# mjuvela/SOC

Measured on AMD Instinct MI355X. Metric: photon packets/sec, higher is better.
Workload: dtype f32

## Files before the change

soc_amd/csrc/soc_brick.hip:

```cpp
#include "soc_walk.h"
#include "soc_ltree.h"

#include <cstdio>
#include <algorithm>
#include <chrono>
#include <cstdlib>
#include <cstring>
#include <vector>

#include "soc_lbricks.h"

#define SOC_BRICK_T 256

#if defined(SOC_BRICK_PROF)
__device__ unsigned long long g_soc_prof[24];
#define SOC_PROF_DECL unsigned int prof_[8] = { 0, 0, 0, 0, 0, 0, 0, 0 }, dprof_[8] = { 0, 0, 0, 0, 0, 0, 0, 0 };  unsigned long long tprof_[8] = { 0, 0, 0, 0, 0, 0, 0, 0 }, tlast_ = __builtin_readcyclecounter()
#define SOC_PROF_T(i) do { const unsigned long long t_ = __builtin_readcyclecounter();  tprof_[i] += t_ - tlast_;  tlast_ = t_; } while (0)
#define SOC_PROF_ENTRY const unsigned long long tentry_ = __builtin_readcyclecounter()
#define SOC_PROF_SINCE_ENTRY(i) do { tprof_[i] += tlast_ - tentry_; } while (0)
#define SOC_PROF(i, n) do { prof_[i] += (unsigned int)(n); } while (0)
#define SOC_DPROF(i, n) do { dprof_[i] += (unsigned int)(n); } while (0)
#define SOC_PROF_FLUSH do { if ((threadIdx.x & 63) == 0) for (int i_ = 0; i_ < 8; i_++) atomicAdd(&g_soc_prof[16 + i_], (unsigned long long)dprof_[i_]); \
                            if ((threadIdx.x & 63) == 0) for (int i_ = 0; i_ < 8; i_++) atomicAdd(&g_soc_prof[i_], (unsigned long long)prof_[i_]); \
                            if ((threadIdx.x & 63) == 0) for (int i_ = 0; i_ < 8; i_++) atomicAdd(&g_soc_prof[8 + i_], tprof_[i_]); } while (0)
// ... 1766 lines not shown
{
    if ((int)blockIdx.x >= nsort) {
        const int e = (int)blockIdx.x - nsort, l = e >> 4, part = e & 15;
        const int start = A.admit[1 + 3 * l], n = A.admit[2 + 3 * l];
        if (n > 0) {
            const int dst = A.admit[3 + 3 * l];
            for (int i = part * SOC_BRICK_T + threadIdx.x; i < n; i += 16 * SOC_BRICK_T) A.idq_next[dst + i] = (uint32_t)(start + i);
        }
        return;
    }
    if ((int)blockIdx.x >= *A.ndesc) return;
    const SocDesc D = A.desc[blockIdx.x];
    for (int j = threadIdx.x; j < D.count; j += SOC_BRICK_T) {
        const uint32_t key = A.keyq[D.start + j];
        if (key < (uint32_t)A.NB) A.idq_next[A.off[key] + A.posq[D.start + j]] = A.idq[D.start + j];
    }
}


#include "soc_devbuf.h"

#define BCHK(call)                          \
    do {                                    \
        hipError_t e_ = (call);             \
        if (e_ != hipSuccess) return e_;    \
    } while (0)

struct SocBrickBuffers {
    DevBuf<SocPk2> pk, park;
    DevBuf<float2> kopt;
    DevBuf<uint32_t> idq[2], keyq, posq;
    DevBuf<SocSimPack> pack;
    DevBuf<int> hist, off, ndesc, total, admit;
    DevBuf<SocDesc> desc[2];
};

template <typename T>
static hipError_t upload(DevBuf<T> &d, const std::vector<T> &v, hipStream_t st)
{
    BCHK(d.reset(v.size(), st));
    return hipMemcpy(d, v.data(), v.size() * sizeof(T), hipMemcpyHostToDevice);
}

struct SocOctBricks {
    bool valid = false;
    int  NB = 0, CAP = 0;
    size_t cells = 0, leaves = 0;
    DevBuf<float2> DS;
    DevBuf<int> bcell, bbase;
};

struct SocLBricksDev {
    bool valid = false, failed = false;
    int  NB = 0, cap = 0, max_slots = 0;
    size_t cells = 0, slots = 0;
    DevBuf<SocLBrick> lbr;
    DevBuf<float> btree;
    DevBuf<int> bcell, bbase, rbrick;
};

struct SocSweepState {
    SocBrickBuffers bb;
    SocOctBricks ob;
    SocLBricksDev lb;
};

SocSweepState *soc_sweep_new() { return new SocSweepState(); }
void soc_sweep_delete(SocSweepState *sw) { delete sw; }
void soc_sweep_invalidate(SocSweepState *sw) { sw->ob.valid = false;  sw->lb.valid = false;  sw->lb.failed = false; }

static hipError_t soc_oct_build(SocOctBricks &ob, const SocGrid &G, int CAP, hipStream_t st, bool verbose)
{
    if (ob.valid && ob.CAP == CAP && ob.cells == (size_t)G.CELLS) return hipSuccess;
    ob.valid = false;
    std::vector<float> D((size_t)G.CELLS);
    BCHK(hipStreamSynchronize(st));
    BCHK(hipMemcpy(D.data(), G.DENS, (size_t)G.CELLS * 4, hipMemcpyDeviceToHost));
    SocOctBuilder B(G.NX, G.NY, G.NZ, G.LEVELS, G.CELLS, G.LCELLS, G.OFF, D.data(), CAP);
    B.build();
    const int NB = (int)B.bbase.size() - 1;
    if (NB < 1 || NB >= (1 << (32 - SOC_SLOT_BITS))) return hipErrorNotSupported;
    std::vector<float2> DS((size_t)G.CELLS);
    for (size_t i = 0; i < (size_t)G.CELLS; i++) { float y;  memcpy(&y, &B.slotmap[i], 4);  DS[i] = make_float2(D[i], y); }
    BCHK(upload(ob.DS, DS, st));
    BCHK(upload(ob.bcell, B.bcell, st));
    BCHK(upload(ob.bbase, B.bbase, st));
    ob.NB = NB;  ob.CAP = CAP;  ob.cells = (size_t)G.CELLS;  ob.leaves = B.bcell.size();
    ob.valid = true;
    if (verbose)
        fprintf(stderr, "soc_brick: hierarchy of %d cells, %zu leaves -> %d bricks of <= %d leaves (mean %.0f)\n",
                G.CELLS, ob.leaves, NB, CAP, (double)ob.leaves / NB);
    return hipSuccess;
}

static hipError_t soc_lb_build(SocLBricksDev &lb, const SocGrid &G, int cap, hipStream_t st, bool verbose)
{
    if (lb.cap == cap && lb.cells == (size_t)G.CELLS) {
        if (lb.valid) return hipSuccess;
        if (lb.failed) return hipErrorNotSupported;
    }
    lb.valid = false;  lb.failed = false;
    lb.cap = cap;  lb.cells = (size_t)G.CELLS;
    std::vector<float> D((size_t)G.CELLS);
    BCHK(hipStreamSynchronize(st));
    BCHK(hipMemcpy(D.data(), G.DENS, (size_t)G.CELLS * 4, hipMemcpyDeviceToHost));
    SocLBricksHost H;
    const bool built = (G.LEVELS == 1) ? soc_cbricks_build(G.NX, G.NY, G.NZ, D.data(), soc_cart_edge(cap), H)
                                       : soc_lbricks_build(G.NX, G.NY, G.NZ, G.LEVELS, G.LCELLS, G.OFF, D.data(), cap, H);
    if (!built || H.bricks.size() >= (1u << 20)) {
        lb.failed = true;
        return hipErrorNotSupported;
    }
    const int NB = (int)H.bricks.size();
    std::vector<int> bbase((size_t)NB + 1);
    for (int b = 0; b < NB; b++) bbase[b] = H.bricks[b].base;
    bbase[NB] = (int)H.btree.size();
    BCHK(upload(lb.lbr, H.bricks, st));
    BCHK(upload(lb.btree, H.btree, st));
    BCHK(upload(lb.bcell, H.bcell, st));
    BCHK(upload(lb.bbase, bbase, st));
    BCHK(upload(lb.rbrick, H.rbrick, st));
    lb.NB = NB;  lb.max_slots = H.max_slots;  lb.slots = H.btree.size();
    lb.valid = true;
    if (verbose)
        fprintf(stderr, "soc_brick: %s of %d cells -> %d brick-local hierarchies of <= %d cells (largest %d, mean %.0f)\n",
                (G.LEVELS == 1) ? "grid" : "hierarchy", G.CELLS, NB, cap, H.max_slots, (double)G.CELLS / NB);
    return hipSuccess;
}


typedef void (*SocPassFn)(const SocGrid, const SocSimPack *, const SocBrickArgs, const int, const int);
static const SocPassFn soc_brick_pass_fns[3][2][2][4] = {
    { { { soc_brick_pass<0, 0, 0, 0, 0>, soc_brick_pass<0, 0, 0, 0, 1>, soc_brick_pass<0, 0, 0, 0, 2>, soc_brick_pass<0, 0, 0, 0, 3> },
        { soc_brick_pass<0, 0, 0, 1, 0>, soc_brick_pass<0, 0, 0, 1, 1>, soc_brick_pass<0, 0, 0, 1, 2>, soc_brick_pass<0, 0, 0, 1, 3> } },
      { { soc_brick_pass<0, 0, 1, 0, 0>, soc_brick_pass<0, 0, 1, 0, 1>, soc_brick_pass<0, 0, 1, 0, 2>, soc_brick_pass<0, 0, 1, 0, 3> },
        { soc_brick_pass<0, 0, 1, 1, 0>, soc_brick_pass<0, 0, 1, 1, 1>, soc_brick_pass<0, 0, 1, 1, 2>, soc_brick_pass<0, 0, 1, 1, 3> } } },
    { { { soc_brick_pass<1, 0, 0, 0, 0>, soc_brick_pass<1, 0, 0, 0, 1>, soc_brick_pass<1, 0, 0, 0, 2>, soc_brick_pass<1, 0, 0, 0, 3> },
        { soc_brick_pass<1, 0, 0, 1, 0>, soc_brick_pass<1, 0, 0, 1, 1>, soc_brick_pass<1, 0, 0, 1, 2>, soc_brick_pass<1, 0, 0, 1, 3> } },
      { { soc_brick_pass<1, 0, 1, 0, 0>, soc_brick_pass<1, 0, 1, 0, 1>, soc_brick_pass<1, 0, 1, 0, 2>, soc_brick_pass<1, 0, 1, 0, 3> },
        { soc_brick_pass<1, 0, 1, 1, 0>, soc_brick_pass<1, 0, 1, 1, 1>, soc_brick_pass<1, 0, 1, 1, 2>, soc_brick_pass<1, 0, 1, 1, 3> } } },
    { { { soc_brick_pass<1, 1, 0, 0, 0>, soc_brick_pass<1, 1, 0, 0, 1>, soc_brick_pass<1, 1, 0, 0, 2>, soc_brick_pass<1, 1, 0, 0, 3> },
        { soc_brick_pass<1, 1, 0, 1, 0>, soc_brick_pass<1, 1, 0, 1, 1>, soc_brick_pass<1, 1, 0, 1, 2>, soc_brick_pass<1, 1, 0, 1, 3> } },
      { { soc_brick_pass<1, 1, 1, 0, 0>, soc_brick_pass<1, 1, 1, 0, 1>, soc_brick_pass<1, 1, 1, 0, 2>, soc_brick_pass<1, 1, 1, 0, 3> },
        { soc_brick_pass<1, 1, 1, 1, 0>, soc_brick_pass<1, 1, 1, 1, 1>, soc_brick_pass<1, 1, 1, 1, 2>, soc_brick_pass<1, 1, 1, 1, 3> } } } };
static const SocPassFn soc_lbrick_pass_fns[4][5] = {
    { soc_lbrick_pass<0, 0>, soc_lbrick_pass<0, 1>, soc_lbrick_pass<0, 2>, soc_lbrick_pass<0, 3>, soc_lbrick_pass<0, 4> },
    { soc_lbrick_pass<1, 0>, soc_lbrick_pass<1, 1>, soc_lbrick_pass<1, 2>, soc_lbrick_pass<1, 3>, soc_lbrick_pass<1, 4> },
    { soc_lbrick_pass<2, 0>, soc_lbrick_pass<2, 1>, soc_lbrick_pass<2, 2>, soc_lbrick_pass<2, 3>, soc_lbrick_pass<2, 4> },
    { soc_lbrick_pass<3, 0>, soc_lbrick_pass<3, 1>, soc_lbrick_pass<3, 2>, soc_lbrick_pass<3, 3>, soc_lbrick_pass<3, 4> } };
static const SocPassFn soc_lbrick_pass_ali_fns[2] = { soc_lbrick_pass_ali<0>, soc_lbrick_pass_ali<1> };
static const SocPassFn soc_lbrick_pass_abu_fns[4] = { soc_lbrick_pass_abu<0>, soc_lbrick_pass_abu<1>, nullptr, soc_lbrick_pass_abu<3> };
static const SocPassFn soc_lbrick_pass_flt_fns[4] = { soc_lbrick_pass_flt<0>, soc_lbrick_pass_flt<1>, soc_lbrick_pass_flt<2>, soc_lbrick_pass_flt<3> };
static const SocPassFn soc_lbrick_pass_ali_flt_fns[2] = { soc_lbrick_pass_ali_flt<0>, soc_lbrick_pass_ali_flt<1> };
static const SocPassFn soc_lray_pass_fns[2][2][2] = { { { soc_lray_pass<0, 0, 0>, soc_lray_pass<0, 1, 0> }, { soc_lray_pass<1, 0, 0>, soc_lray_pass<1, 1, 0> } },
                                                      { { soc_lray_pass<0, 0, 1>, soc_lray_pass<0, 1, 1> }, { soc_lray_pass<1, 0, 1>, soc_lray_pass<1, 1, 1> } } };

static const SocPassFn soc_lray_pass_flt_fns[2][2] = { { soc_lray_pass<0, 0, 0, 1>, soc_lray_pass<0, 1, 0, 1> }, { soc_lray_pass<1, 0, 0, 1>, soc_lray_pass<1, 1, 0, 1> } };

static SocPassFn pass_kernel(const SocSweepPlan &pl)
{
    const bool flt = (pl.form == 3) && pl.octree && !pl.dbl;
    if (pl.rays)      return flt ? soc_lray_pass_flt_fns[pl.hpx][pl.hpsky] : soc_lray_pass_fns[pl.octree ? 0 : 1][pl.hpx][pl.hpsky];
    if (flt && pl.abu) return nullptr;
    if (flt)          return pl.ali ? soc_lbrick_pass_ali_flt_fns[pl.wint] : soc_lbrick_pass_flt_fns[pl.wint];
    if (pl.form == 3 && pl.abu) return soc_lbrick_pass_abu_fns[pl.wint];
    if (pl.form == 3) return pl.ali ? soc_lbrick_pass_ali_fns[pl.wint] : soc_lbrick_pass_fns[pl.wint][pl.kind];
    return soc_brick_pass_fns[pl.octree + pl.dbl][pl.abu][pl.wint][pl.kind];
}

static hipError_t check_sca(const SocSim *S, int nlaunch, const SocVariant &V, const SocSca *sca)
{
    if (!sca) return hipSuccess;
    if (sca->NDIR == 0 || V.abu || V.wint) return hipErrorNotSupported;
    for (int l = 0; l < nlaunch; l++) {
        const int k = S[l].SCAKIND - 1;
        if ((k != SOC_SCA_PB && k != SOC_SCA_PS && k != SOC_SCA_CL && k != SOC_SCA_HP) || S[l].NDUST > 1 || S[l].BINS < 1 || !S[l].OUT) return hipErrorNotSupported;
        if ((k == SOC_SCA_PB || k == SOC_SCA_PS) && !S[l].DSC) return hipErrorNotSupported;
        if ((k == SOC_SCA_HP) && (!S[l].HPBG || (S[l].HPBG_WEIGHTED && !S[l].HPBGP))) return hipErrorNotSupported;
        if ((k == SOC_SCA_CL) != (S[l].SOURCE == SOC_SOURCE_CL)) return hipErrorInvalidValue;
    }
    return hipSuccess;
}

static hipError_t plan_sweep(SocSweepPlan &pl, const SocGrid &G, const SocSim *S, int nlaunch, const SocVariant &V,
                             const SocBrickTune &tune, const SocSca *sca, bool lb_ok)
{
    const bool cart = lb_ok && sca && soc_brick_cart(G, V);
    bool xab = false;
    for (int l = 0; l < nlaunch; l++) xab = xab || (S[l].XAB != nullptr);
    const bool lt = cart || (lb_ok && soc_brick_local(G, V, tune) && !(V.abu && xab));
    pl = soc_grid_plan(lt ? 3 : V.octree ? 2 : 1, 0, V);
    pl.rays = sca != nullptr;
    pl.hpx = sca && sca->NDIR < 0;
    for (int l = 0; l < nlaunch && sca; l++) pl.hpsky = pl.hpsky || (S[l].SCAKIND == SOC_SCA_HP + 1);
    const auto pick = [](int t, int d) { return (t > 0) ? t : d; };
    pl.T = pick(tune.T, 512);
    if (lt) {
        pl.P = pick(tune.P, 16384);
        pl.KCAP = pick(tune.KCAP, 64);
        pl.FTH = pick(tune.FTH, 16);
        pl.CTH = pick(tune.CTH, 8);
        pl.TAIL = pick(tune.TAIL, 32);
        pl.PARK = pick(tune.park, 4096);
        pl.slow_every = tune.slow_every;
    } else {
        pl.P = pick(tune.P, V.octree ? 4096 : 2048);
        pl.KCAP = pick(tune.KCAP, V.octree ? 32 : 48);
        pl.FTH = pick(tune.FTH, V.octree ? 16 : 24);
        pl.CTH = pick(tune.CTH, pl.FTH);
        pl.TAIL = pick(tune.TAIL, 0);
        pl.CAP = pick(tune.CAP, 6144);
    }
    if (pl.T < 64 || pl.T > 1024 || (pl.T & 63) || pl.P < 1 || pl.P > SOC_LBRICK_PMAX || pl.KCAP < 1) return hipErrorInvalidValue;
    pl.EQ = 2;
    if (!lt) {
        if (sca || V.wint == 2) return hipErrorNotSupported;
        for (int l = 0; l < nlaunch; l++) if (S[l].ROISAVE) return hipErrorNotSupported;
        if (pl.T > 512 || pl.P > SOC_BRICK_PMAX || pl.CAP < 8 || pl.CAP > (1 << SOC_SLOT_BITS)) return hipErrorInvalidValue;
        return hipSuccess;
    }
    bool int_only = !sca && (V.wint == 1);
    for (int l = 0; l < nlaunch && int_only; l++)
        for (int m = 0; m < l; m++) if (S[m].INT == S[l].INT && S[m].TW != S[l].TW) { int_only = false;  break; }
    bool ali = !sca && (V.wint != 2);
    for (int l = 0; l < nlaunch; l++) ali = ali && (S[l].SOURCE == SOC_SOURCE_CL) && (S[l].XAB != nullptr) && (S[l].XAB == S[0].XAB);
    if (ali) int_only = false;
    pl.wint = int_only ? 3 : V.wint;
    pl.ali = ali;
    const int cedge = soc_cart_default_edge(G);
    const int cap_abu = (V.wint && !int_only) ? 3456 : 4352;
    pl.capl = (tune.CAP > 0) ? tune.CAP : cart ? cedge * cedge * cedge : (sca ? 17408 : V.abu ? cap_abu : (ali ? (V.wint ? 3456 : 4352) : (V.wint == 2 ? 2944 : (V.wint && !int_only) ? 5888 : 8704)));
    if (pl.capl < 8 || pl.capl > 36864) return hipErrorInvalidValue;
    pl.EQ = 3;
    for (int l = 0; l < nlaunch; l++) pl.roi = pl.roi || (S[l].ROISAVE && S[l].ROI);
    if (pl.roi) {
        for (int l = 0; l < nlaunch; l++) if (!(S[l].ROISAVE && S[l].ROI) || S[l].MIRROR) return hipErrorNotSupported;
        pl.EQ = 4;
    }
    return hipSuccess;
}

static hipError_t build_bricks(SocBrickArgs &A, const SocSweepPlan &pl, SocSweepState &sw, const SocGrid &G, int LB, hipStream_t st, bool verbose)
{
    A = SocBrickArgs{};
    A.LB = LB;
    A.ev_brick = -1;
    A.T = pl.T;  A.P = pl.P;  A.KCAP = pl.KCAP;  A.FTH = pl.FTH;  A.CTH = pl.CTH;  A.CAP = pl.CAP;  A.TAIL = pl.TAIL;  A.PARK = pl.PARK;
    A.EQ = pl.EQ;  A.slow_every = pl.slow_every;
    A.LT = (pl.form == 3);  A.int_only = (pl.wint == 3);  A.ali = pl.ali;  A.roi_on = pl.roi;
    if (pl.form == 1) {
        const int B = 1 << LB;
        A.NBX = (G.NX + B - 1) / B;  A.NBY = (G.NY + B - 1) / B;  A.NBZ = (G.NZ + B - 1) / B;
        A.NB = A.NBX * A.NBY * A.NBZ;
        return (A.NB > (1 << 18)) ? hipErrorNotSupported : hipSuccess;
    }
    int k = 1;
    while ((1 << k) <= std::max(G.NX, std::max(G.NY, G.NZ))) k++;
    A.sib_thr = ldexpf(1.0f, k - 29);
    A.kexp = k - 30;
    if (pl.form == 3) {
        BCHK(soc_lb_build(sw.lb, G, pl.capl, st, verbose));
        const SocLBricksDev &lb = sw.lb;
        A.NB = lb.NB;
        A.CAP = (lb.max_slots + 63) & ~63;
        A.lbr = lb.lbr;  A.btree = lb.btree;  A.bcell = lb.bcell;  A.bbase = lb.bbase;  A.rbrick = lb.rbrick;
        A.kopt_stride = pl.abu ? (long long)lb.slots : 0;
        return hipSuccess;
    }
    if (G.LEVELS > 15) return hipErrorNotSupported;
    BCHK(soc_oct_build(sw.ob, G, A.CAP, st, verbose));
    const SocOctBricks &ob = sw.ob;
    A.NB = ob.NB;
    A.DS = ob.DS;  A.bcell = ob.bcell;  A.bbase = ob.bbase;
    return hipSuccess;
}

struct SocSweepSize {
    uint32_t count;
    int NQ;
    int maxdesc;
};

static hipError_t pack_launches(SocSimPack &K, SocSweepSize &sz, SocBrickArgs &A, const SocSweepPlan &pl, const SocGrid &G,
                                const SocSim *Sin, int nlaunch, const SocBrickTune &tune)
{
    uint32_t count = 0;
    for (int l = 0; l < nlaunch; l++) {
        const SocSim &S = Sin[l];
        if (S.BATCH >= (1 << 24)) return hipErrorNotSupported;
        uint32_t c = S.gid_count;
        if ((S.SOURCE == 1 || S.SOURCE == SOC_SOURCE_HP) && S.SCAKIND != SOC_SCA_HP + 1 && !tune.oversub) {
            const long long lim = 8LL * 2 * ((long long)G.NX * G.NY + (long long)G.NY * G.NZ + (long long)G.NZ * G.NX);
            if ((long long)S.gid0 >= lim) c = 0;
            else if ((long long)S.gid0 + c > lim) c = (uint32_t)(lim - S.gid0);
        }
        if (S.SOURCE == 3) {
            if (S.ROILOAD < 1 || !S.ROI) return hipErrorNotSupported;
            const long long lim = 100LL * S.ROILOAD;
            if ((long long)S.gid0 >= lim) c = 0;
            else if ((long long)S.gid0 + c > lim) c = (uint32_t)(lim - S.gid0);
        }
        if (S.SOURCE == SOC_SOURCE_CL) {
            if ((long long)S.gid0 >= G.CELLS) c = 0;
            else if ((long long)S.gid0 + c > G.CELLS) c = (uint32_t)(G.CELLS - S.gid0);
            if (S.USE_EMWEIGHT == 2) return hipErrorNotSupported;
            if (S.XAB && !pl.ali) return hipErrorNotSupported;
        }
        if (S.BATCH <= 0 && S.SOURCE != SOC_SOURCE_CL) c = 0;
        if (c == 0) continue;
        if ((unsigned long long)count + c > 0x7fffffffull) return hipErrorNotSupported;
        K.S[K.n] = S;
        K.S[K.n].gid_count = c;
        K.first[K.n] = count;
        count += c;
        K.n++;
    }
    for (int l = K.n; l <= SOC_MAXLAUNCH; l++) K.first[l] = count;
    if (pl.abu && pl.form != 3 && K.n > 1) {
        A.opt_stride = (long long)(K.S[1].OPT - K.S[0].OPT);
        for (int l = 1; l < K.n; l++)
            if ((long long)(K.S[l].OPT - K.S[0].OPT) != l * A.opt_stride) return hipErrorInvalidValue;
    }
    const bool by_int = pl.wint != 0, by_opt = pl.abu && pl.form == 3;
    int ngrp = 0;
    for (int l = 0; l < K.n; l++) {
        int g = 0;
        while (g < ngrp && ((by_int && K.S[K.gfirst[g]].INT != K.S[l].INT) || (by_opt && K.S[K.gfirst[g]].OPT != K.S[l].OPT))) g++;
        if (g == ngrp) K.gfirst[ngrp++] = l;
        K.grp[l] = g;
    }
    A.NBQ = (ngrp > 1) ? A.NB * ngrp : A.NB;
    if ((long long)A.NB * ngrp > (1 << 20)) return hipErrorNotSupported;
    A.nl = K.n;
    sz.count = count;
    sz.NQ = A.NBQ + A.EQ * K.n + 1;
    return hipSuccess;
}

static hipError_t plan_kernel(SocSweepPlan &pl, SocBrickArgs &A, SocSweepSize &sz, const SocSimPack &K, const SocBrickTune &tune)
{
    const long long pop = (pl.form == 3) ? 600000000LL : pl.octree ? 26000000LL : std::max(2700000LL, 5300LL * A.NBQ);
    A.target = (int)std::min<long long>((tune.POP > 0) ? tune.POP : std::min(pop, 2000000000LL), sz.count);
    sz.maxdesc = (int)(((uint32_t)A.target + A.P - 1) / A.P) + sz.NQ + K.n;
    A.HS = (sz.NQ > 4096) ? 1024 : 0;
    if (tune.HS > 0) A.HS = tune.HS;
    if (A.HS & (A.HS - 1)) return hipErrorInvalidValue;
    const int BV = (pl.octree || pl.form == 3) ? A.CAP : (1 << (3 * A.LB));
    const int nh = A.HS ? 2 * A.HS : sz.NQ;
    const size_t lds_walk = (pl.form == 3) ? (size_t)(BV * (pl.rays ? 1 : (2 + (pl.wint == 2 ? 4 : (pl.wint == 1) ? 1 : 0) + (pl.ali ? 2 : 0) + (pl.abu ? 2 : 0)))
                                                      + ((nh + 3) & ~3) + 4 + 4 * SOC_MAXLAUNCH) * 4
                                           : (size_t)(BV * (1 + pl.wint) + nh + 2 + 3 * SOC_MAXLAUNCH + SOC_MAXL + A.P) * 4;
    const size_t lds_ev = (size_t)(nh + 4 + SOC_MAXL) * 4;
    pl.lds = std::max(lds_walk, lds_ev);
    if (pl.lds > 160 * 1024) return hipErrorNotSupported;
    if (!pl.rays) {
        bool several = false, all_bg = true;
        pl.kind = soc_source_kind(K.S[0].SOURCE);
        for (int l = 0; l < K.n; l++) {
            several = several || (soc_source_kind(K.S[l].SOURCE) != pl.kind);
            all_bg = all_bg && (K.S[l].SOURCE == 1);
        }
        if (several && pl.form != 3) return hipErrorInvalidValue;
        if (several) pl.kind = 4;
        else if (all_bg && !tune.nolean) pl.kind = 3;
        if (pl.form == 3 && pl.abu) pl.kind = 4;
        if (pl.form == 3 && pl.octree && !pl.dbl) pl.kind = pl.ali ? 2 : 4;
    }
    if (pl.form == 3 && pl.abu && (pl.wint == 2 || pl.ali)) return hipErrorNotSupported;
    if (pl.form != 3) for (int l = 0; l < K.n; l++) if (K.S[l].MIRROR) return hipErrorNotSupported;
    return hipSuccess;
}

static hipError_t reserve_buffers(SocBrickBuffers &bb, SocBrickArgs &A, const SocSweepSize &sz, const SocSca *sca, hipStream_t st)
{
    BCHK(bb.pk.reserve(sz.count, st));
    for (DevBuf<uint32_t> *q : { &bb.idq[0], &bb.idq[1], &bb.keyq, &bb.posq }) BCHK(q->reserve(sz.count, st));
    BCHK(bb.hist.reserve(sz.NQ, st));
    BCHK(bb.off.reserve(sz.NQ, st));
    BCHK(bb.desc[0].reserve(sz.maxdesc, st));
    BCHK(bb.desc[1].reserve(sz.maxdesc, st));
    if (sca) {
        BCHK(bb.park.reserve(sz.count, st));
        A.park = bb.park;
        A.sca = *sca;
    }
    if (A.LT && A.kopt_stride > 0) {
        BCHK(bb.kopt.reserve((size_t)(A.NBQ / A.NB) * (size_t)A.kopt_stride, st));
        A.kopt = bb.kopt;
    }
    BCHK(bb.pack.reserve(1, st));
    BCHK(bb.ndesc.reserve(4, st));
    BCHK(bb.total.reserve(1, st));
    BCHK(bb.admit.reserve(1 + 3 * SOC_MAXLAUNCH, st));
    A.pk = bb.pk;  A.keyq = bb.keyq;  A.posq = bb.posq;  A.hist = bb.hist;  A.off = bb.off;  A.total = bb.total;
    A.admit = bb.admit;
    A.first = (const uint32_t *)((const char *)bb.pack.p + offsetof(SocSimPack, first));
    return hipSuccess;
// ... 87 lines not shown
```

soc_amd/csrc/soc_capi.hip:

```cpp
#include "soc_host.h"
#include "soc_rng.h"

#include <cmath>
#include <cstdarg>
#include <cstdio>
#include <cstring>
#include <functional>

#define SOC_HPBG_PIX 49152

std::atomic<int64_t> soc_dev_bytes{0};

static std::string g_create_err;

int fail(soc_ctx *c, int code, const char *fmt, ...)
{
    char buf[512];
    va_list ap;
    va_start(ap, fmt);
    vsnprintf(buf, sizeof buf, fmt, ap);
    va_end(ap);
    if (c) c->err = buf;
    else   g_create_err = buf;
    return code;
// ... 244 lines not shown
int soc_set_features(soc_ctx *c, int with_int, int ps_method, int use_emweight)
{
    if (!c) return SOC_ERR_ARG;
    FLUSH(c);
    if (!(ps_method == 0 || ps_method == 1 || ps_method == 2 || ps_method == 4 || ps_method == 5))
        return fail(c, SOC_ERR_ARG, "soc_set_features: PS_METHOD %d not supported (0,1,2,4,5)", ps_method);
    if (use_emweight < 0 || use_emweight > 2)
        return fail(c, SOC_ERR_ARG, "soc_set_features: USE_EMWEIGHT %d not supported (0,1,2)", use_emweight);
    if (with_int == 2) {
        if (!c->have_grid) return fail(c, SOC_ERR_STATE, "soc_set_features: with_int 2 needs soc_set_grid first (it allocates INTX, INTY, INTZ)");
        HIPCHK(c, hipSetDevice(c->device));
        if (c->dINTV.n != (size_t)3 * c->G.CELLS) {
            HIPCHK(c, hipStreamSynchronize(c->stream));
            HIPCHK(c, c->dINTV.reset((size_t)3 * c->G.CELLS, c->stream));
            HIPCHK(c, hipMemsetAsync(c->dINTV, 0, (size_t)3 * c->G.CELLS * 4, c->stream));
        }
    }
    c->with_int = (with_int == 2) ? 2 : (with_int ? 1 : 0);
    c->ps_method = ps_method;
    c->use_emweight = use_emweight;
    return SOC_OK;
}

int soc_set_mirror(soc_ctx *c, int mask)
{
    if (!c) return SOC_ERR_ARG;
    FLUSH(c);
    if (mask < 0 || mask > 63) return fail(c, SOC_ERR_ARG, "soc_set_mirror: mask %d (bits x,X,y,Y,z,Z = 1,2,4,8,16,32)", mask);
    c->mirror = mask;
    return SOC_OK;
}

int soc_set_exec(soc_ctx *c, int mode, int brick_log2)
{
    if (!c) return SOC_ERR_ARG;
    FLUSH(c);
    if (mode < -1 || mode > 1 || brick_log2 < 2 || brick_log2 > 4)
        return fail(c, SOC_ERR_ARG, "soc_set_exec: mode %d (-1,0,1), brick_log2 %d (2..4)", mode, brick_log2);
    c->exec_mode = mode;
    c->brick_log2 = brick_log2;
    return SOC_OK;
}

int soc_set_tuning(soc_ctx *c, const char *name, int value)
{
    if (!c || !name) return SOC_ERR_ARG;
    FLUSH(c);
    if (value < 0) return fail(c, SOC_ERR_ARG, "soc_set_tuning: %s = %d (0 = built-in choice)", name, value);
    struct { const char *n; int *p; } tab[] = {
        { "threads", &c->tune.T }, { "chunk", &c->tune.P }, { "steps_per_visit", &c->tune.KCAP }, { "swap_lanes", &c->tune.FTH },
        { "climb_lanes", &c->tune.CTH }, { "brick_cells", &c->tune.CAP }, { "tail_lanes", &c->tune.TAIL }, { "park_below", &c->tune.park }, { "population", &c->tune.POP },
        { "hash_slots", &c->tune.HS }, { "global_tree", &c->tune.global_tree }, { "slow_every", &c->tune.slow_every },
        { "general_kernel", &c->tune.nolean }, { "oversubscribe", &c->tune.oversub }, { "verbose", &c->tune.verbose },
        { "abu_local", &c->tune.abu_local }, { "float_local", &c->tune.float_local } };
    for (auto &t : tab)
        if (!strcmp(name, t.n)) {
            if (t.p == &c->tune.CAP && value != c->tune.CAP) soc_sweep_invalidate(c->sweep);
            *t.p = value;
            return SOC_OK;
        }
    return fail(c, SOC_ERR_ARG, "soc_set_tuning: unknown parameter '%s'", name);
}

int soc_last_passes(soc_ctx *c) { return c ? c->last.passes : 0; }
int soc_last_form(soc_ctx *c) { return (c && c->last.passes > 0) ? c->last.form : 0; }
int soc_last_variant(soc_ctx *c) { return c ? c->last.variant : -1; }

int soc_set_optical(soc_ctx *c, const float *ABS, const float *SCA, int ndust)
{
    if (!c) return SOC_ERR_ARG;
    if (!ABS || !SCA || ndust != 1) return fail(c, SOC_ERR_ARG, "soc_set_optical: need ABS, SCA with ndust==1 (WITH_MSF is not supported)");
    c->ABS = ABS[0];
    c->SCA = SCA[0];
    c->have_optical = true;
    return SOC_OK;
}

int soc_set_opt(soc_ctx *c, const float *OPT)
{
    if (!c) return SOC_ERR_ARG;
    if (!c->have_grid) return fail(c, SOC_ERR_STATE, "soc_set_opt: call soc_set_grid first");
    HIPCHK(c, hipSetDevice(c->device));
    c->opt_from_abu = false;
    c->opt_gen++;
    if (!OPT) {
        HIPCHK(c, hipStreamSynchronize(c->stream));
        c->dOPT.release();
        return SOC_OK;
    }
    if (!c->dOPT) HIPCHK(c, c->dOPT.reset((size_t)c->G.CELLS, c->stream));
    HIPCHK(c, hipMemcpyAsync(c->dOPT, OPT, (size_t)c->G.CELLS * 8, hipMemcpyHostToDevice, c->stream));
    if (c->opt_half) HIPCHK(c, soc_launch_opt_half(c->G.CELLS, c->dOPT, c->stream));
    HIPCHK(c, hipStreamSynchronize(c->stream));
    return SOC_OK;
}

int soc_set_opt_half(soc_ctx *c, int on)
{
    if (!c) return SOC_ERR_ARG;
    c->opt_half = on != 0;
    return SOC_OK;
}

int soc_set_abundances(soc_ctx *c, int NDUST, int single, const float *ABU)
{
    if (!c) return SOC_ERR_ARG;
    FLUSH(c);
    if (!c->have_grid) return fail(c, SOC_ERR_STATE, "soc_set_abundances: call soc_set_grid first");
    HIPCHK(c, hipSetDevice(c->device));
    c->opt_from_abu = false;
// ... 1071 lines not shown
```

soc_amd/csrc/soc_dev.h:

```cpp
#ifndef SOC_DEV_H
#define SOC_DEV_H

#include <hip/hip_runtime.h>
#include <stdint.h>
#include <algorithm>

#define SOC_MAXL 16

struct SocGrid {
    int NX, NY, NZ, LEVELS, CELLS, NXYZ;
    int OFF[SOC_MAXL];
    int LCELLS[SOC_MAXL];
    const float *DENS;
    const int   *PAR;
};

struct SocRoi {
    int   save, load;
    int   ROI[6];
    int   STEP, NSIDE;
    int   DIM[3], NELEM;
    float *SAVE;
    const float *LOAD;
};
// ... 204 lines not shown
#define SOC_A2E_LDS (160 * 1024)
bool soc_a2e_shape(int NE, int NFREQ, int out[3]);
hipError_t soc_launch_a2e_dosolve(const SocA2EArgs &A, hipStream_t st);
hipError_t soc_launch_a2e_eqtemp(const SocEqTArgs &A, hipStream_t st);
hipError_t soc_launch_eqsolver(const SocEqTArgs &A, hipStream_t st);

#define SOC_MABU_LDS (64 * 1024)
hipError_t soc_launch_mabu_split(long long cells, int NFREQ, int NDUST, int idust, const float *ABS, const float *ABU, const double *RABS,
                                 float *PART, hipStream_t st);
hipError_t soc_launch_mabu_clip(long long cells, int NFREQ, float *PART, hipStream_t st);
hipError_t soc_launch_mabu_sum(long long cells, int NFREQ, int NDUST, int idust, const float *EM, const float *ABU, float *SUM, hipStream_t st);
hipError_t soc_launch_mabu_poleq(long long cells, int NFREQ, int NA, const float *EM, const float *AALG, const double *APOL, const double *TAB,
                                 float *PEM, hipStream_t st);
hipError_t soc_launch_mabu_ratio(long long cells, int NFREQ, const float *SUM, float *PSUM, hipStream_t st);

struct SocLibSolve {
    long long    n;
    int          N, nout;
    float        I0, dI0;
    const float *I1, *dI1;
    const float *I2, *dI2;
    const float *X, *Y, *Z;
    const float *E0;
    const float *E;
    const float *ABS;
    long long    stride;
    int          c0, c1, c2;
    float       *EMI;
    int         *miss;
    unsigned long long *nmiss;
};
struct SocLibBuild {
    long long    cells;
    int          N;
    const float *ABS;
    long long    stride;
    int          c0, c1, c2;
    float        I0, dI0;
    const float *I1, *dI1, *I2, *dI2;
};
hipError_t soc_launch_library_solve(const SocLibSolve &A, hipStream_t st);
hipError_t soc_launch_library_range(const SocLibBuild &A, int level, unsigned *TAB, hipStream_t st);
hipError_t soc_launch_library_pick(const SocLibBuild &A, unsigned long long *BEST, int *IND, float *XX, float *YY, float *ZZ, hipStream_t st);

struct SocBrickTune {
    int T, P, KCAP, FTH, CTH, CAP, TAIL, POP, HS;
    int global_tree;
    int park;
    int slow_every;
    int nolean;
    int oversub;
    int verbose;
    int abu_local;
    int float_local;
};

static inline int soc_source_kind(int source) { return (source == SOC_SOURCE_CL) ? 2 : (source == SOC_SOURCE_HP) ? 1 : 0; }

static inline SocVariant soc_grid_variant(const SocGrid &G, bool abu = false, int wint = 0)
{
    SocVariant V;
    V.octree = G.LEVELS > 1;
    V.dbl = G.NX > ((G.LEVELS < 3) ? 399 : 100);
    V.abu = abu;
    V.wint = wint;
    return V;
}

static inline bool soc_brick_local(const SocGrid &G, const SocVariant &V, const SocBrickTune &tune)
{
    const int n = std::max(G.NX, std::max(G.NY, G.NZ));
    return V.octree && (V.dbl || (tune.float_local && !V.abu)) && (!V.abu || (tune.abu_local && V.wint != 2)) && !tune.global_tree && G.LEVELS <= 8 && ((long long)n << (G.LEVELS - 1)) < (1LL << 24) && n < 4096;
}

static inline bool soc_brick_cart(const SocGrid &G, const SocVariant &V)
{
    const int n = std::max(G.NX, std::max(G.NY, G.NZ));
    return !V.octree && !V.abu && G.LEVELS == 1 && n < 4096 && ((long long)G.NY * G.NZ) < (1LL << 23);
}
#define SOC_CART_BRICK_EDGE 16
#define SOC_CART_BRICK_EDGE_WIDE 24
#define SOC_CART_BRICK_WIDE 256
static inline int soc_cart_default_edge(const SocGrid &G)
{
    return (std::max(G.NX, std::max(G.NY, G.NZ)) >= SOC_CART_BRICK_WIDE) ? SOC_CART_BRICK_EDGE_WIDE : SOC_CART_BRICK_EDGE;
}
static inline int soc_cart_edge(int cells)
{
    int e = 1;
    while ((long long)(e + 1) * (e + 1) * (e + 1) <= cells) e++;
    return e;
}

struct SocSweepPlan {
    int  form;
    int  kind;
    int  wint;
    bool octree, dbl, abu;
    bool ali;
    bool rays, hpx, hpsky;
    bool roi;
    int  capl;
    int  T, P, KCAP, FTH, CTH, CAP, TAIL, PARK, EQ, slow_every;
    size_t lds;
};

static inline SocSweepPlan soc_grid_plan(int form, int kind, const SocVariant &V)
{
    SocSweepPlan p{};
    p.form = form;
    p.kind = kind;
    p.wint = V.wint ? 1 : 0;
    p.octree = V.octree;
    p.dbl = V.octree && V.dbl;
    p.abu = V.abu;
    return p;
}

#define SOC_VAR_HEALPIX (1 << 12)
#define SOC_VAR_HPSKY   (1 << 13)
static inline int soc_variant_code(const SocSweepPlan &p)
{
    return p.form | (p.kind << 2) | (p.wint << 5) | (p.octree ? 1 << 7 : 0) | (p.dbl ? 1 << 8 : 0) | (p.abu ? 1 << 9 : 0) | (p.ali ? 1 << 10 : 0)
           | (p.rays ? 1 << 11 : 0) | (p.hpx ? SOC_VAR_HEALPIX : 0) | (p.hpsky ? SOC_VAR_HPSKY : 0);
}

struct SocSweepResult {
    int passes = 0, form = 0, variant = -1;
};

struct SocSweepState;
SocSweepState *soc_sweep_new();
void soc_sweep_delete(SocSweepState *sw);
void soc_sweep_invalidate(SocSweepState *sw);
hipError_t soc_brick_run_pb(SocSweepState &sw, const SocGrid &G, const SocSim *S, int nlaunch, const SocVariant &V, int LB,
                            const SocBrickTune &tune, hipStream_t st, SocSweepResult *res, const struct SocSca *sca = nullptr);

#endif
```

soc_amd/csrc/soc_lbricks.h:

```cpp
#ifndef SOC_LBRICKS_H
#define SOC_LBRICKS_H

#include <cstdint>
#include <cstring>
#include <vector>

#include "soc_ltree.h"

struct SocLBricksHost {
    std::vector<SocLBrick> bricks;
    std::vector<float>     btree;
    std::vector<int>       bcell;
    std::vector<int>       rbrick;
    int  max_slots = 0;
    bool ok = false;
};

namespace soc_lb {

inline int link_of(float d) { float m = -d;  int i;  memcpy(&i, &m, 4);  return i; }
inline float link_to(int i) { float m;  memcpy(&m, &i, 4);  return -m; }

struct Builder {
    int NX, NY, NZ, LEVELS, cap;
    const int *LCELLS, *OFF;
    const float *D;
    std::vector<uint32_t> sub;
    SocLBricksHost &out;

    Builder(int nx, int ny, int nz, int levels, const int *lcells, const int *off, const float *dens, int cap_, SocLBricksHost &o)
        : NX(nx), NY(ny), NZ(nz), LEVELS(levels), cap(cap_), LCELLS(lcells), OFF(off), D(dens), out(o) {}

    bool count()
    {
        std::vector<uint32_t> below, cur;
        for (int l = LEVELS - 1; l >= 0; l--) {
            cur.assign((size_t)LCELLS[l], 1u);
            const float *d = D + OFF[l];
            for (int i = 0; i < LCELLS[l]; i++) {
                if (d[i] > 0.0f) continue;
                if (l + 1 >= LEVELS) return false;
                const int c = link_of(d[i]);
                if (c < 0 || c + 8 > LCELLS[l + 1]) return false;
                uint64_t n = 1;
                for (int k = 0; k < 8; k++) n += below[(size_t)c + k];
                cur[i] = (uint32_t)(n > 0x7fffffffu ? 0x7fffffffu : n);
            }
            below.swap(cur);
        }
        sub.swap(below);
        return true;
    }
    uint64_t cells_in(int x0, int y0, int z0, int dx, int dy, int dz) const
    {
        uint64_t n = 0;
        for (int z = z0; z < z0 + dz; z++)
            for (int y = y0; y < y0 + dy; y++) {
                const uint32_t *row = sub.data() + ((size_t)z * NY + y) * NX;
                for (int x = x0; x < x0 + dx; x++) n += row[x];
            }
        return n;
    }
    bool emit(int x0, int y0, int z0, int dx, int dy, int dz, int n)
    {
        SocLBrick K;
        K.x0 = x0;  K.y0 = y0;  K.z0 = z0;  K.bx = dx;  K.by = dy;  K.bz = dz;
        K.base = (int)out.btree.size();
        K.nslot = n;
        const int id = (int)out.bricks.size();
        const size_t base = out.btree.size();
        out.btree.resize(base + n);
        out.bcell.resize(base + n);
        std::vector<int> lev((size_t)n);
        int fill = 0;
        for (int z = z0; z < z0 + dz; z++)
            for (int y = y0; y < y0 + dy; y++)
                for (int x = x0; x < x0 + dx; x++) {
                    const int r = (z * NY + y) * NX + x;
                    out.rbrick[r] = id;
                    out.bcell[base + fill] = r;
                    lev[fill] = 0;
                    fill++;
                }
        for (int s = 0; s < fill; s++) {
            const int g = out.bcell[base + s];
            const float d = D[g];
            if (d > 0.0f) { out.btree[base + s] = d;  continue; }
            if (fill + 8 > n) return false;
            const int l = lev[s], c = OFF[l + 1] + link_of(d);
            out.btree[base + s] = link_to(fill);
            for (int k = 0; k < 8; k++) { out.bcell[base + fill] = c + k;  lev[fill] = l + 1;  fill++; }
        }
        if (fill != n) return false;
        out.bricks.push_back(K);
        if (n > out.max_slots) out.max_slots = n;
        return true;
    }
    bool split(int x0, int y0, int z0, int dx, int dy, int dz)
    {
        const uint64_t n = cells_in(x0, y0, z0, dx, dy, dz);
        if (n <= (uint64_t)cap) return emit(x0, y0, z0, dx, dy, dz, (int)n);
        if (dx == 1 && dy == 1 && dz == 1) return false;
        if (dz >= dy && dz >= dx) { const int h = (dz + 1) / 2;  return split(x0, y0, z0, dx, dy, h) && split(x0, y0, z0 + h, dx, dy, dz - h); }
        if (dy >= dx)             { const int h = (dy + 1) / 2;  return split(x0, y0, z0, dx, h, dz) && split(x0, y0 + h, z0, dx, dy - h, dz); }
        const int h = (dx + 1) / 2;
        return split(x0, y0, z0, h, dy, dz) && split(x0 + h, y0, z0, dx - h, dy, dz);
    }
    bool build()
    {
        out = SocLBricksHost();
        if (!count()) return false;
        out.rbrick.assign((size_t)NX * NY * NZ, -1);
        size_t total = 0;
        for (int l = 0; l < LEVELS; l++) total += (size_t)LCELLS[l];
        out.btree.reserve(total);
        out.bcell.reserve(total);
        const int T = 16;
        for (int z = 0; z < NZ; z += T)
            for (int y = 0; y < NY; y += T)
                for (int x = 0; x < NX; x += T) {
                    const int dx = (x + T <= NX) ? T : NX - x, dy = (y + T <= NY) ? T : NY - y, dz = (z + T <= NZ) ? T : NZ - z;
                    if (!split(x, y, z, dx, dy, dz)) return false;
                }
        out.ok = true;
        return true;
    }
};

}

inline bool soc_lbricks_build(int NX, int NY, int NZ, int LEVELS, const int *LCELLS, const int *OFF, const float *DENS, int cap,
                              SocLBricksHost &out)
{
    soc_lb::Builder B(NX, NY, NZ, LEVELS, LCELLS, OFF, DENS, cap, out);
    const bool ok = B.build();
    if (!ok) out = SocLBricksHost();
    return ok;
}

inline bool soc_cbricks_build(int NX, int NY, int NZ, const float *DENS, int edge, SocLBricksHost &out)
{
    out = SocLBricksHost();
    if (NX < 1 || NY < 1 || NZ < 1 || edge < 1) return false;
    const size_t cells = (size_t)NX * NY * NZ;
    for (size_t i = 0; i < cells; i++) if (!(DENS[i] > 0.0f)) return false;
    out.rbrick.assign(cells, -1);
    out.btree.resize(cells);
    out.bcell.resize(cells);
    size_t fill = 0;
    for (int z0 = 0; z0 < NZ; z0 += edge)
        for (int y0 = 0; y0 < NY; y0 += edge)
            for (int x0 = 0; x0 < NX; x0 += edge) {
                SocLBrick K;
                K.x0 = x0;  K.y0 = y0;  K.z0 = z0;
                K.bx = (x0 + edge <= NX) ? edge : NX - x0;  K.by = (y0 + edge <= NY) ? edge : NY - y0;  K.bz = (z0 + edge <= NZ) ? edge : NZ - z0;
                K.base = (int)fill;
                K.nslot = K.bx * K.by * K.bz;
                const int id = (int)out.bricks.size();
                for (int z = z0; z < z0 + K.bz; z++)
                    for (int y = y0; y < y0 + K.by; y++)
                        for (int x = x0; x < x0 + K.bx; x++) {
                            const size_t r = ((size_t)z * NY + y) * NX + x;
                            out.rbrick[r] = id;
                            out.bcell[fill] = (int)r;
                            out.btree[fill] = DENS[r];
                            fill++;
                        }
                out.bricks.push_back(K);
                if (K.nslot > out.max_slots) out.max_slots = K.nslot;
            }
    out.ok = true;
    return true;
}

#endif
```

Baseline: 465.3 million.

## Partition hierarchy into slab/column bricks minimizing total face area

Adds a density-aware recursive partitioner that cuts the refined grid into slabs and columns sized to the brick cap. It tries several axis orders and piece counts, scores each by total brick surface area, and keeps whichever of this and the old fixed 16^3 tiling has less face area. Less face area should mean fewer photon crossings between bricks and less cross-brick queueing. It also lowers the hash-slot threshold, adds a tuning switch to force the old tiles, and makes the host-side build slower.

```diff
diff --git a/soc_amd/csrc/soc_brick.hip b/soc_amd/csrc/soc_brick.hip
--- a/soc_amd/csrc/soc_brick.hip
+++ b/soc_amd/csrc/soc_brick.hip
@@ -1842,6 +1842,7 @@
 
 struct SocLBricksDev {
     bool valid = false, failed = false;
+    bool tiles = false;
     int  NB = 0, cap = 0, max_slots = 0;
     size_t cells = 0, slots = 0;
     DevBuf<SocLBrick> lbr;
@@ -1883,20 +1884,22 @@
     return hipSuccess;
 }
 
-static hipError_t soc_lb_build(SocLBricksDev &lb, const SocGrid &G, int cap, hipStream_t st, bool verbose)
-{
-    if (lb.cap == cap && lb.cells == (size_t)G.CELLS) {
+static hipError_t soc_lb_build(SocLBricksDev &lb, const SocGrid &G, int cap, bool tiles, hipStream_t st, bool verbose)
+{
+    if (lb.cap == cap && lb.tiles == tiles && lb.cells == (size_t)G.CELLS) {
         if (lb.valid) return hipSuccess;
         if (lb.failed) return hipErrorNotSupported;
     }
     lb.valid = false;  lb.failed = false;
-    lb.cap = cap;  lb.cells = (size_t)G.CELLS;
+    lb.cap = cap;  lb.tiles = tiles;  lb.cells = (size_t)G.CELLS;
     std::vector<float> D((size_t)G.CELLS);
     BCHK(hipStreamSynchronize(st));
     BCHK(hipMemcpy(D.data(), G.DENS, (size_t)G.CELLS * 4, hipMemcpyDeviceToHost));
     SocLBricksHost H;
+    const auto t0 = std::chrono::steady_clock::now();
     const bool built = (G.LEVELS == 1) ? soc_cbricks_build(G.NX, G.NY, G.NZ, D.data(), soc_cart_edge(cap), H)
-                                       : soc_lbricks_build(G.NX, G.NY, G.NZ, G.LEVELS, G.LCELLS, G.OFF, D.data(), cap, H);
+                                       : soc_lbricks_build(G.NX, G.NY, G.NZ, G.LEVELS, G.LCELLS, G.OFF, D.data(), cap, H, tiles ? SOC_LB_TILES : SOC_LB_BEST);
+    const double secs = std::chrono::duration<double>(std::chrono::steady_clock::now() - t0).count();
     if (!built || H.bricks.size() >= (1u << 20)) {
         lb.failed = true;
         return hipErrorNotSupported;
@@ -1912,9 +1915,14 @@
     BCHK(upload(lb.rbrick, H.rbrick, st));
     lb.NB = NB;  lb.max_slots = H.max_slots;  lb.slots = H.btree.size();
     lb.valid = true;
-    if (verbose)
-        fprintf(stderr, "soc_brick: %s of %d cells -> %d brick-local hierarchies of <= %d cells (largest %d, mean %.0f)\n",
-                (G.LEVELS == 1) ? "grid" : "hierarchy", G.CELLS, NB, cap, H.max_slots, (double)G.CELLS / NB);
+    if (verbose) {
+        double area = 0.0;
+        for (const SocLBrick &K : H.bricks) area += 2.0 * ((double)K.bx * K.by + (double)K.by * K.bz + (double)K.bz * K.bx);
+        fprintf(stderr, "soc_brick: %s of %d cells -> %d brick-local hierarchies of <= %d cells (largest %d, mean %.0f, fill %.3f), face area %.4g",
+                (G.LEVELS == 1) ? "grid" : "hierarchy", G.CELLS, NB, cap, H.max_slots, (double)G.CELLS / NB, (double)G.CELLS / NB / cap, area);
+        if (G.LEVELS > 1) fprintf(stderr, " (%s; tiles %.4g, slabs %.4g)", H.slabs ? "slabs" : "tiles", H.area_tiles, H.area_slabs);
+        fprintf(stderr, ", built in %.2f s\n", secs);
+    }
     return hipSuccess;
 }
 
@@ -2021,6 +2029,7 @@
     const int cap_abu = (V.wint && !int_only) ? 3456 : 4352;
     pl.capl = (tune.CAP > 0) ? tune.CAP : cart ? cedge * cedge * cedge : (sca ? 17408 : V.abu ? cap_abu : (ali ? (V.wint ? 3456 : 4352) : (V.wint == 2 ? 2944 : (V.wint && !int_only) ? 5888 : 8704)));
     if (pl.capl < 8 || pl.capl > 36864) return hipErrorInvalidValue;
+    pl.tiles = (tune.partition == 1);
     pl.EQ = 3;
     for (int l = 0; l < nlaunch; l++) pl.roi = pl.roi || (S[l].ROISAVE && S[l].ROI);
     if (pl.roi) {
@@ -2049,7 +2058,7 @@
     A.sib_thr = ldexpf(1.0f, k - 29);
     A.kexp = k - 30;
     if (pl.form == 3) {
-        BCHK(soc_lb_build(sw.lb, G, pl.capl, st, verbose));
+        BCHK(soc_lb_build(sw.lb, G, pl.capl, pl.tiles, st, verbose));
         const SocLBricksDev &lb = sw.lb;
         A.NB = lb.NB;
         A.CAP = (lb.max_slots + 63) & ~63;
@@ -2132,7 +2141,7 @@
     const long long pop = (pl.form == 3) ? 600000000LL : pl.octree ? 26000000LL : std::max(2700000LL, 5300LL * A.NBQ);
     A.target = (int)std::min<long long>((tune.POP > 0) ? tune.POP : std::min(pop, 2000000000LL), sz.count);
     sz.maxdesc = (int)(((uint32_t)A.target + A.P - 1) / A.P) + sz.NQ + K.n;
-    A.HS = (sz.NQ > 4096) ? 1024 : 0;
+    A.HS = (sz.NQ > 2048) ? 1024 : 0;
     if (tune.HS > 0) A.HS = tune.HS;
     if (A.HS & (A.HS - 1)) return hipErrorInvalidValue;
     const int BV = (pl.octree || pl.form == 3) ? A.CAP : (1 << (3 * A.LB));
diff --git a/soc_amd/csrc/soc_capi.hip b/soc_amd/csrc/soc_capi.hip
--- a/soc_amd/csrc/soc_capi.hip
+++ b/soc_amd/csrc/soc_capi.hip
@@ -320,10 +320,12 @@
         { "climb_lanes", &c->tune.CTH }, { "brick_cells", &c->tune.CAP }, { "tail_lanes", &c->tune.TAIL }, { "park_below", &c->tune.park }, { "population", &c->tune.POP },
         { "hash_slots", &c->tune.HS }, { "global_tree", &c->tune.global_tree }, { "slow_every", &c->tune.slow_every },
         { "general_kernel", &c->tune.nolean }, { "oversubscribe", &c->tune.oversub }, { "verbose", &c->tune.verbose },
-        { "abu_local", &c->tune.abu_local }, { "float_local", &c->tune.float_local } };
+        { "abu_local", &c->tune.abu_local }, { "float_local", &c->tune.float_local }, { "brick_partition", &c->tune.partition } };
     for (auto &t : tab)
         if (!strcmp(name, t.n)) {
+            if (t.p == &c->tune.partition && value > 2) return fail(c, SOC_ERR_ARG, "soc_set_tuning: brick_partition = %d (0 built-in, 1 tiles, 2 smallest face area)", value);
             if (t.p == &c->tune.CAP && value != c->tune.CAP) soc_sweep_invalidate(c->sweep);
+            if (t.p == &c->tune.partition && (value == 1) != (c->tune.partition == 1)) soc_sweep_invalidate(c->sweep);
             *t.p = value;
             return SOC_OK;
         }
diff --git a/soc_amd/csrc/soc_dev.h b/soc_amd/csrc/soc_dev.h
--- a/soc_amd/csrc/soc_dev.h
+++ b/soc_amd/csrc/soc_dev.h
@@ -280,6 +280,7 @@
     int oversub;
     int verbose;
     int abu_local;
+    int partition;
     int float_local;
 };
 
@@ -329,6 +330,7 @@
     bool rays, hpx, hpsky;
     bool roi;
     int  capl;
+    bool tiles;
     int  T, P, KCAP, FTH, CTH, CAP, TAIL, PARK, EQ, slow_every;
     size_t lds;
 };
diff --git a/soc_amd/csrc/soc_lbricks.h b/soc_amd/csrc/soc_lbricks.h
--- a/soc_amd/csrc/soc_lbricks.h
+++ b/soc_amd/csrc/soc_lbricks.h
@@ -1,6 +1,8 @@
 #ifndef SOC_LBRICKS_H
 #define SOC_LBRICKS_H
 
+#include <algorithm>
+#include <cmath>
 #include <cstdint>
 #include <cstring>
 #include <vector>
@@ -14,7 +16,18 @@
     std::vector<int>       rbrick;
     int  max_slots = 0;
     bool ok = false;
+    double area_tiles = 0.0, area_slabs = 0.0;
+    int    n_tiles = 0, n_slabs = 0;
+    bool   slabs = false;
 };
+
+enum { SOC_LB_BEST = 0, SOC_LB_TILES = 1 };
+#ifndef SOC_LB_SKEW
+#define SOC_LB_SKEW 2.0
+#endif
+#ifndef SOC_LB_NODE
+#define SOC_LB_NODE 4096
+#endif
 
 namespace soc_lb {
 
@@ -96,32 +109,249 @@
         if (n > out.max_slots) out.max_slots = n;
         return true;
     }
-    bool split(int x0, int y0, int z0, int dx, int dy, int dz)
+    struct Box { int x0, y0, z0, dx, dy, dz;  uint32_t n; };
+    typedef std::vector<Box> Boxes;
+
+    static double area(const Boxes &B)
+    {
+        double a = 0.0;
+        for (const Box &b : B) a += 2.0 * ((double)b.dx * b.dy + (double)b.dy * b.dz + (double)b.dz * b.dx);
+        return a;
+    }
+    static Box sub_box(const Box &b, int axis, int a0, int a1, uint64_t n)
+    {
+        Box c = b;
+        if (axis == 0) { c.x0 = b.x0 + a0;  c.dx = a1 - a0; } else if (axis == 1) { c.y0 = b.y0 + a0;  c.dy = a1 - a0; } else { c.z0 = b.z0 + a0;  c.dz = a1 - a0; }
+        c.n = (uint32_t)(n > 0xffffffffu ? 0xffffffffu : n);
+        return c;
+    }
+
+    bool split(int x0, int y0, int z0, int dx, int dy, int dz, Boxes &B) const
     {
         const uint64_t n = cells_in(x0, y0, z0, dx, dy, dz);
-        if (n <= (uint64_t)cap) return emit(x0, y0, z0, dx, dy, dz, (int)n);
+        if (n <= (uint64_t)cap) { B.push_back(Box{ x0, y0, z0, dx, dy, dz, (uint32_t)n });  return true; }
         if (dx == 1 && dy == 1 && dz == 1) return false;
-        if (dz >= dy && dz >= dx) { const int h = (dz + 1) / 2;  return split(x0, y0, z0, dx, dy, h) && split(x0, y0, z0 + h, dx, dy, dz - h); }
-        if (dy >= dx)             { const int h = (dy + 1) / 2;  return split(x0, y0, z0, dx, h, dz) && split(x0, y0 + h, z0, dx, dy - h, dz); }
+        if (dz >= dy && dz >= dx) { const int h = (dz + 1) / 2;  return split(x0, y0, z0, dx, dy, h, B) && split(x0, y0, z0 + h, dx, dy, dz - h, B); }
+        if (dy >= dx)             { const int h = (dy + 1) / 2;  return split(x0, y0, z0, dx, h, dz, B) && split(x0, y0 + h, z0, dx, dy - h, dz, B); }
         const int h = (dx + 1) / 2;
-        return split(x0, y0, z0, h, dy, dz) && split(x0 + h, y0, z0, dx - h, dy, dz);
-    }
-    bool build()
+        return split(x0, y0, z0, h, dy, dz, B) && split(x0 + h, y0, z0, dx - h, dy, dz, B);
+    }
+    bool tiles(Boxes &B) const
+    {
+        const int T = 16;
+        for (int z = 0; z < NZ; z += T)
+            for (int y = 0; y < NY; y += T)
+                for (int x = 0; x < NX; x += T) {
+                    const int dx = (x + T <= NX) ? T : NX - x, dy = (y + T <= NY) ? T : NY - y, dz = (z + T <= NZ) ? T : NZ - z;
+                    if (!split(x, y, z, dx, dy, dz, B)) return false;
+                }
+        return true;
+    }
+
+    void profile(const Box &b, int axis, std::vector<uint64_t> &P) const
+    {
+        const int len = (axis == 0) ? b.dx : (axis == 1) ? b.dy : b.dz;
+        P.assign((size_t)len + 1, 0);
+        for (int z = 0; z < b.dz; z++)
+            for (int y = 0; y < b.dy; y++) {
+                const uint32_t *row = sub.data() + ((size_t)(b.z0 + z) * NY + (b.y0 + y)) * NX + b.x0;
+                if (axis == 0) for (int x = 0; x < b.dx; x++) P[x + 1] += row[x];
+                else { uint64_t n = 0;  for (int x = 0; x < b.dx; x++) n += row[x];  P[(axis == 1 ? y : z) + 1] += n; }
+            }
+        for (int i = 0; i < len; i++) P[i + 1] += P[i];
+    }
+    static int nearest(const std::vector<uint64_t> &P, int lo, int hi, double want)
+    {
+        int a = lo, b = hi;
+        while (a < b) { const int m = (a + b) / 2;  if ((double)P[m] < want) a = m + 1; else b = m; }
+        if (a > lo && want - (double)P[a - 1] <= (double)P[a] - want) a--;
+        return a;
+    }
+    static void even_cuts(const std::vector<uint64_t> &P, int k, std::vector<int> &C)
+    {
+        const int len = (int)P.size() - 1;
+        C.assign(1, 0);
+        for (int i = 1; i < k; i++) C.push_back(nearest(P, C.back() + 1, len - (k - i), (double)P[len] * i / k));
+        C.push_back(len);
+    }
+    void capped_cuts(const std::vector<uint64_t> &P, std::vector<int> &C) const
+    {
+        const int len = (int)P.size() - 1;
+        std::vector<int> G(1, 0);
+        while (G.back() < len) {
+            int c = G.back() + 1;
+            while (c < len && P[c + 1] - P[G.back()] <= (uint64_t)cap) c++;
+            G.push_back(c);
+        }
+        const int k = (int)G.size() - 1;
+        C.assign(1, 0);
+        bool fits = true;
+        for (int i = 1; i < k && fits; i++) {
+            const int lo = C.back() + 1, hi = len - (k - i);
+            if (lo > hi) { fits = false;  break; }
+            int c = nearest(P, lo, hi, (double)P[len] * i / k);
+            while (c > lo && P[c] - P[C.back()] > (uint64_t)cap) c--;
+            if (P[c] - P[C.back()] > (uint64_t)cap) fits = false;
+            C.push_back(c);
+        }
+        C.push_back(len);
+        const int m = (int)C.size();
+        if (!fits || m != k + 1 || (P[len] - P[C[m - 2]] > (uint64_t)cap && len - C[m - 2] > 1)) C = G;
+    }
+    static int len_of(const Box &b, int axis) { return (axis == 0) ? b.dx : (axis == 1) ? b.dy : b.dz; }
+    static double area_rest(const Boxes &R)
+    {
+        double a = 0.0;
+        for (const Box &r : R) a += 4.0 * ((double)r.dx * r.dy + (double)r.dy * r.dz + (double)r.dz * r.dx);
+        return a;
+    }
+    static void piece_counts(int len, double e, double shrink, int &k0, int &k1)
+    {
+        const double r = (double)len / e;
+        k0 = std::min(len, std::max(1, (int)std::floor(r)));
+        k1 = std::min(len, std::max(k0, (int)std::ceil(r / shrink)));
+    }
+    void column_cut(const Box &c, int ax, Boxes &B, Boxes &rest) const
+    {
+        if (c.n <= (uint32_t)cap) { B.push_back(c);  return; }
+        std::vector<uint64_t> P;
+        std::vector<int> C;
+        profile(c, ax, P);
+        capped_cuts(P, C);
+        for (size_t i = 0; i + 1 < C.size(); i++) {
+            const Box x = sub_box(c, ax, C[i], C[i + 1], P[C[i + 1]] - P[C[i]]);
+            (x.n <= (uint32_t)cap ? B : rest).push_back(x);
+        }
+    }
+    void columns_cut(const Box &s, int ay, int ax, Boxes &B, Boxes &rest) const
+    {
+        if (s.n <= (uint32_t)cap) { B.push_back(s);  return; }
+        std::vector<uint64_t> P;
+        std::vector<int> C;
+        profile(s, ay, P);
+        int k0, k1;
+        piece_counts(len_of(s, ay), std::sqrt((double)cap * len_of(s, ay) * len_of(s, ax) / (double)s.n), std::sqrt(0.75), k0, k1);
+        Boxes T, R, bestT, bestR;
+        double abest = -1.0;
+        for (int k = k0; k <= k1; k++) {
+            T.clear();  R.clear();
+            even_cuts(P, k, C);
+            for (size_t i = 0; i + 1 < C.size(); i++) column_cut(sub_box(s, ay, C[i], C[i + 1], P[C[i + 1]] - P[C[i]]), ax, T, R);
+            const double a = area(T) + area_rest(R);
+            if (abest < 0.0 || a < abest) { abest = a;  bestT.swap(T);  bestR.swap(R); }
+        }
+        B.insert(B.end(), bestT.begin(), bestT.end());
+        rest.insert(rest.end(), bestR.begin(), bestR.end());
+    }
+    double slab_cut(const Box &b, int az, int ay, int ax, Boxes &B, Boxes &rest) const
+    {
+        std::vector<uint64_t> P;
+        std::vector<int> C;
+        profile(b, az, P);
+        int k0, k1;
+        piece_counts(len_of(b, az), std::cbrt((double)cap * b.dx * b.dy * b.dz / (double)b.n), std::cbrt(0.75), k0, k1);
+        Boxes T, R;
+        double abest = -1.0;
+        for (int k = k0; k <= k1; k++) {
+            T.clear();  R.clear();
+            even_cuts(P, k, C);
+            for (size_t i = 0; i + 1 < C.size(); i++) columns_cut(sub_box(b, az, C[i], C[i + 1], P[C[i + 1]] - P[C[i]]), ay, ax, T, R);
+            const double a = area(T) + area_rest(R);
+            if (abest < 0.0 || a < abest) { abest = a;  B.swap(T);  rest.swap(R); }
+        }
+        return abest;
+    }
+    bool part(const Box &b, Boxes &B) const
+    {
+        if (b.n <= (uint32_t)cap) { B.push_back(b);  return true; }
+        if (b.dx == 1 && b.dy == 1 && b.dz == 1) return false;
+        const int axis = (b.dz >= b.dy && b.dz >= b.dx) ? 2 : (b.dy >= b.dx) ? 1 : 0;
+        const int len = len_of(b, axis);
+        if ((uint64_t)b.n > (uint64_t)SOC_LB_NODE * (uint64_t)cap) {
+            std::vector<uint64_t> P;
+            profile(b, axis, P);
+            const int c = nearest(P, 1, len - 1, 0.5 * (double)P[len]);
+            return part(sub_box(b, axis, 0, c, P[c]), B) && part(sub_box(b, axis, c, len, P[len] - P[c]), B);
+        }
+        {
+            const int hx = (b.dx + 1) / 2, hy = (b.dy + 1) / 2, hz = (b.dz + 1) / 2;
+            uint64_t oct[8] = { 0, 0, 0, 0, 0, 0, 0, 0 };
+            for (int z = 0; z < b.dz; z++)
+                for (int y = 0; y < b.dy; y++) {
+                    const uint32_t *row = sub.data() + ((size_t)(b.z0 + z) * NY + (b.y0 + y)) * NX + b.x0;
+                    uint64_t *o = oct + ((z >= hz) ? 4 : 0) + ((y >= hy) ? 2 : 0);
+                    for (int x = 0; x < hx; x++) o[0] += row[x];
+                    for (int x = hx; x < b.dx; x++) o[1] += row[x];
+                }
+            double lo = 0.0, hi = 0.0;
+            uint64_t nlo = 0;
+            for (int k = 0; k < 8; k++) {
+                const double v = (double)((k & 1) ? b.dx - hx : hx) * ((k & 2) ? b.dy - hy : hy) * ((k & 4) ? b.dz - hz : hz);
+                if (!((k >> axis) & 1)) nlo += oct[k];
+                if (v <= 0.0) continue;
+                const double rho = (double)oct[k] / v;
+                if (hi == 0.0 || rho > hi) hi = rho;
+                if (lo == 0.0 || rho < lo) lo = rho;
+            }
+            if (hi > SOC_LB_SKEW * lo) {
+                const int h = (len + 1) / 2;
+                return part(sub_box(b, axis, 0, h, nlo), B) && part(sub_box(b, axis, h, len, (uint64_t)b.n - nlo), B);
+            }
+        }
+        static const int ORD[6][3] = { { 2, 1, 0 }, { 2, 0, 1 }, { 1, 2, 0 }, { 1, 0, 2 }, { 0, 2, 1 }, { 0, 1, 2 } };
+        const double e = std::cbrt((double)cap * b.dx * b.dy * b.dz / (double)b.n);
+        const int nord = ((double)std::min(b.dx, std::min(b.dy, b.dz)) < 3.0 * e) ? 6 : 1;
+        Boxes best, bestrest, T, R;
+        double abest = -1.0;
+        for (int o = 0; o < nord; o++) {
+            T.clear();  R.clear();
+            const double a = slab_cut(b, ORD[o][0], ORD[o][1], ORD[o][2], T, R);
+            bool same = false;
+            for (const Box &r : R) same = same || (r.dx == b.dx && r.dy == b.dy && r.dz == b.dz);
+            if (same) continue;
+            if (abest < 0.0 || a < abest) { abest = a;  best.swap(T);  bestrest.swap(R); }
+        }
+        if (abest < 0.0) {
+            const int h = (len + 1) / 2;
+            const Box lo = sub_box(b, axis, 0, h, 0);
+            const uint64_t nlo = cells_in(lo.x0, lo.y0, lo.z0, lo.dx, lo.dy, lo.dz);
+            return part(sub_box(b, axis, 0, h, nlo), B) && part(sub_box(b, axis, h, len, (uint64_t)b.n - nlo), B);
+        }
+        B.insert(B.end(), best.begin(), best.end());
+        for (const Box &r : bestrest) if (!part(r, B)) return false;
+        return true;
+    }
+    bool slabs(Boxes &B) const
+    {
+        const uint64_t n = cells_in(0, 0, 0, NX, NY, NZ);
+        if (n > 0xffffffffu) return false;
+        return part(Box{ 0, 0, 0, NX, NY, NZ, (uint32_t)n }, B);
+    }
+
+    bool boxes(int partition, Boxes &B)
     {
         out = SocLBricksHost();
         if (!count()) return false;
+        Boxes S;
+        if (!tiles(B)) return false;
+        out.area_tiles = area(B);  out.n_tiles = (int)B.size();
+        if (partition != SOC_LB_TILES && slabs(S)) {
+            out.area_slabs = area(S);  out.n_slabs = (int)S.size();
+            out.slabs = out.area_slabs < out.area_tiles;
+        }
+        if (out.slabs) B.swap(S);
+        return true;
+    }
+    bool build(int partition)
+    {
+        Boxes B;
+        if (!boxes(partition, B)) return false;
         out.rbrick.assign((size_t)NX * NY * NZ, -1);
         size_t total = 0;
         for (int l = 0; l < LEVELS; l++) total += (size_t)LCELLS[l];
         out.btree.reserve(total);
         out.bcell.reserve(total);
-        const int T = 16;
-        for (int z = 0; z < NZ; z += T)
-            for (int y = 0; y < NY; y += T)
-                for (int x = 0; x < NX; x += T) {
-                    const int dx = (x + T <= NX) ? T : NX - x, dy = (y + T <= NY) ? T : NY - y, dz = (z + T <= NZ) ? T : NZ - z;
-                    if (!split(x, y, z, dx, dy, dz)) return false;
-                }
+        for (const Box &b : B) if (!emit(b.x0, b.y0, b.z0, b.dx, b.dy, b.dz, (int)b.n)) return false;
         out.ok = true;
         return true;
     }
@@ -130,10 +360,10 @@
 }
 
 inline bool soc_lbricks_build(int NX, int NY, int NZ, int LEVELS, const int *LCELLS, const int *OFF, const float *DENS, int cap,
-                              SocLBricksHost &out)
+                              SocLBricksHost &out, int partition = SOC_LB_BEST)
 {
     soc_lb::Builder B(NX, NY, NZ, LEVELS, LCELLS, OFF, DENS, cap, out);
-    const bool ok = B.build();
+    const bool ok = B.build(partition);
     if (!ok) out = SocLBricksHost();
     return ok;
 }
```

Measured after the change: 493.3 million (median of 6 runs). +6.0%, better.
